# Alibaba-Gemini-Lab/Gemini-SEAL

Hardware: AMD Instinct MI355X
Metric: ciphertext multiply+relinearize/s (BFV N=2^15, 8 primes, bit-exact PARITY mode) (higher is better)
Workload: dtype u64

## Files before the change

gemini-seal_amd/csrc/devmath.hpp:

```cpp
#pragma once

#include <hip/hip_runtime.h>

#include <cstdint>
#include "ntt_bounds.hpp"

namespace sealhip
{
    using u64 = unsigned long long;

    struct PrimeDev
    {
        u64 p;
        u64 two_p;
        u64 rdp;
        u64 cr0, cr1;
        u64 inv_n, inv_n_shoup;
        u64 inv_n_w, inv_n_w_shoup;
        u64 ninv;
        const u64 *fwd;
        const u64 *inv;
        const double *fwd_d;
        const double *inv_d;
        double p_d, pinv_d;
    };

    constexpr double kTwo52 = 4503599627370496.0;
    __device__ __forceinline__ double fp_of(u64 bits)
    {
        return __longlong_as_double(static_cast<long long>(bits));
    }
    __device__ __forceinline__ u64 fp_bits(double v)
    {
        return static_cast<u64>(__double_as_longlong(v));
    }
    __device__ __forceinline__ double fp_from_u64(u64 x)
    {
        return fp_of(x | 0x4330000000000000ull) - kTwo52;
    }
    __device__ __forceinline__ u64 fp_to_u64(double r)
    {
        return fp_bits(r + kTwo52) & 0x000FFFFFFFFFFFFFull;
    }
    __device__ __forceinline__ double fp_reduce(double x, double p, double pinv)
    {
#pragma clang fp contract(off)
        return __builtin_fma(-__builtin_rint(x * pinv), p, x);
    }
    __device__ __forceinline__ double fp_canonical(double x, double p, double pinv)
    {
        const double r = fp_reduce(x, p, pinv);
        return r < 0.0 ? r + p : r;
    }
    __device__ __forceinline__ double fp_mulmod(double y, double w, double p, double pinv)
    {
#pragma clang fp contract(off)
        const double h = y * w;
        const double l = __builtin_fma(y, w, -h);
// ... 162 lines not shown
                : "v"(x0), "s"(s1), "v"(A)
                : "vcc");
        else
            asm("v_mad_u64_u32 %0, vcc, %2, %3, %4\n\ts_nop 1\n\tv_cndmask_b32_e64 %1, 0, 1, vcc"
                : "=&v"(B), "=&v"(cb)
                : "v"(x0), "v"(s1), "v"(A)
                : "vcc");
        const u64 addend = static_cast<u64>(static_cast<u32>(B >> 32)) | (static_cast<u64>(cb) << 32);
        return mad64<SU>(x1, s1, addend);
    }
    __device__ __forceinline__ u64 add_hi32(u64 v, u64 e)
    {
        u32 vh;
        asm("v_add_u32 %0, %1, %2" : "=v"(vh) : "v"(static_cast<u32>(v >> 32)), "v"(static_cast<u32>(e)));
        return static_cast<u64>(static_cast<u32>(v)) | (static_cast<u64>(vh) << 32);
    }
    template <bool WU>
    __device__ __forceinline__ u64 mullo2_acc(u64 acc, u64 x, u64 w, u64 q, u64 np)
    {
        const u32 x0 = static_cast<u32>(x), x1 = static_cast<u32>(x >> 32);
        const u32 w0 = static_cast<u32>(w), w1 = static_cast<u32>(w >> 32);
        const u32 q0 = static_cast<u32>(q), q1 = static_cast<u32>(q >> 32);
        const u32 n0 = static_cast<u32>(np), n1 = static_cast<u32>(np >> 32);
        u64 E = mul64<WU>(x0, w1);
        E = mad64<WU>(x1, w0, E);
        E = mad64<true>(q0, n1, E);
        E = mad64<true>(q1, n0, E);
        u64 V = mad64<WU>(x0, w0, acc);
        V = mad64<true>(q0, n0, V);
        return add_hi32(V, E);
    }
    __device__ __forceinline__ u64 mullo1_acc(u64 acc, u64 q, u64 np)
    {
        const u32 q0 = static_cast<u32>(q), q1 = static_cast<u32>(q >> 32);
        const u32 n0 = static_cast<u32>(np), n1 = static_cast<u32>(np >> 32);
        u64 E = mul64<true>(q0, n1);
        E = mad64<true>(q1, n0, E);
        return add_hi32(mad64<true>(q0, n0, acc), E);
    }
    template <bool WU>
    __device__ __forceinline__ u64 mulmod_lazy_hs(u64 x, u64 y, u64 yshoup, u64 neg_p)
    {
        return mullo2_acc<WU>(0, x, y, mulhi_c<WU>(x, yshoup), neg_p);
    }
    __device__ __forceinline__ u64 mulmod_shoup_hs(u64 x, u64 y, u64 yshoup, u64 p)
    {
        const u64 t = mulmod_lazy_hs<true>(x, y, yshoup, 0 - p);
        return t >= p ? t - p : t;
    }
    __device__ __forceinline__ u64 barrett_lazy_hs(u64 x, u64 rdp, u64 neg_p)
    {
        return mullo1_acc(x, mulhi_c<true>(x, rdp), neg_p);
    }
    __device__ __forceinline__ float small_quot_const(u64 p)
    {
        return static_cast<float>(4294967296.0 / static_cast<double>(p) * (1.0 - 0x1p-20));
    }
    __device__ __forceinline__ u64 reduce_small_quot(u64 x, float c, u64 neg_p)
    {
        float hf;
        asm("v_cvt_f32_u32 %0, %1" : "=v"(hf) : "v"(static_cast<u32>(x >> 32)));
        const u32 q = static_cast<u32>(hf * c);
        const u64 v = mad64<true>(q, static_cast<u32>(neg_p), x);
        return add_hi32(v, static_cast<u64>(q * static_cast<u32>(neg_p >> 32)));
    }
    template <bool SU>
    __device__ __forceinline__ u64 mulhi_apx(u64 x, u64 s)
    {
        const u32 x0 = static_cast<u32>(x), x1 = static_cast<u32>(x >> 32);
        const u32 s0 = static_cast<u32>(s), s1 = static_cast<u32>(s >> 32);
        const u64 A = mul64<SU>(x1, s0);
        u64 B;
        u32 cb;
        if (SU)
            asm("v_mad_u64_u32 %0, vcc, %2, %3, %4\n\ts_nop 1\n\tv_cndmask_b32_e64 %1, 0, 1, vcc"
                : "=&v"(B), "=&v"(cb)
                : "v"(x0), "s"(s1), "v"(A)
                : "vcc");
        else
            asm("v_mad_u64_u32 %0, vcc, %2, %3, %4\n\ts_nop 1\n\tv_cndmask_b32_e64 %1, 0, 1, vcc"
                : "=&v"(B), "=&v"(cb)
                : "v"(x0), "v"(s1), "v"(A)
                : "vcc");
        const u64 addend = static_cast<u64>(static_cast<u32>(B >> 32)) | (static_cast<u64>(cb) << 32);
        return mad64<SU>(x1, s1, addend);
    }
    template <int N>
    struct ZeroHi
    {
        u64 z[N];
        __device__ __forceinline__ void init()
        {
#pragma unroll
            for (int j = 0; j < N; j++)
            {
                u32 h;
                asm volatile("v_mov_b32 %0, 0" : "=v"(h));
                z[j] = static_cast<u64>(h) << 32;
            }
        }
    };
    __device__ __forceinline__ u64 with_low(u64 zp, u32 lo)
    {
        return (zp & 0xFFFFFFFF00000000ull) | lo;
    }
    template <bool SU>
// ... 351 lines not shown
```

gemini-seal_amd/csrc/engine.cpp:

```cpp
#include "engine.hpp"

#include <algorithm>
#include <atomic>
#include <cstdlib>
#include <cstring>

namespace sealhip
{
    namespace
    {
        template <class T>
        T *upload(Engine &e, std::vector<void *> &owned, const T *host, std::size_t count)
        {
            T *dev = nullptr;
            SEALHIP_CHECK(hipMalloc(reinterpret_cast<void **>(&dev), sizeof(T) * (count ? count : 1)));
            owned.push_back(dev);
            if (count)
                SEALHIP_CHECK(hipMemcpy(dev, host, sizeof(T) * count, hipMemcpyHostToDevice));
            (void)e;
            return dev;
        }

        RowMap make_map(const std::vector<unsigned short> &ids)
        {
// ... 477 lines not shown
                const u64 b = hr.Bsk[j];
                const HostNttTables &tb = tables[n_key + (j < B ? 2 + j : 0)];
                if (tb.p != b)
                    throw std::logic_error("internal: Bsk prime order");
                rd.floor_G1m_top[0][j] = mont(mulmod(rd.floor_G1[j], tb.inv_n, b), b);
                rd.floor_G1m_top[1][j] = mont(mulmod(rd.floor_G1[j], tb.inv_n_w, b), b);
                rd.floor_G1m_top[2][j] = mont(rd.floor_G1m_top[0][j], b);
                rd.floor_G1m_top[3][j] = mont(rd.floor_G1m_top[1][j], b);
                rd.b_p[j] = b;
                rd.b_w1[j] = tb.fwd.size() >= 4 ? tb.fwd[2] : 0;
                rd.b_w1s[j] = tb.fwd.size() >= 4 ? tb.fwd[3] : 0;
                rd.b_rdp[j] = tb.rdp ? tb.rdp : shoup(1, b);
                {
                    u64 inv = b;
                    for (int it = 0; it < 6; it++)
                        inv *= 2 - b * inv;
                    rd.b_ninv[j] = 0 - inv;
                }
            }
            for (int i = 0; i < k; i++)
            {
                const u64 qi = hr.q[i];
                rd.floor_F0_top[0][i] = mulmod(rd.floor_F0[i], tables[i].inv_n, qi);
                rd.floor_F0_top[1][i] = mulmod(rd.floor_F0[i], tables[i].inv_n_w, qi);
                rd.floor_F0_top_s[0][i] = shoup(rd.floor_F0_top[0][i], qi);
                rd.floor_F0_top_s[1][i] = shoup(rd.floor_F0_top[1][i], qi);
                for (int hh = 0; hh < 2; hh++)
                {
                    rd.floor_F0_top[2 + hh][i] = mont(rd.floor_F0_top[hh][i], qi);
                    rd.floor_F0_top_s[2 + hh][i] = shoup(rd.floor_F0_top[2 + hh][i], qi);
                }
                rd.q_p[i] = qi;
                rd.q_rdp[i] = tables[i].rdp ? tables[i].rdp : shoup(1, qi);
                {
                    u64 inv = qi;
                    for (int it = 0; it < 6; it++)
                        inv *= 2 - qi * inv;
                    rd.q_ninv[i] = 0 - inv;
                }
                rd.q_mt_inv_s[i] = shoup(rd.q_mt_inv[i], qi);
                rd.floor_F0_s[i] = shoup(rd.floor_F0[i], qi);
                rd.pBm[i] = mont(hr.prod_B_mod_q[i], qi);
                rd.nBm[i] = mont(qi - hr.prod_B_mod_q[i], qi);
                for (int j = 0; j < B; j++)
                    BQm[static_cast<std::size_t>(i) * B + j] = mont(hr.B_to_q.matrix[static_cast<std::size_t>(i) * B + j], qi);
            }
            for (int j = 0; j < B; j++)
                rd.B_to_mskm[j] = mont(hr.B_to_m_sk.matrix[j], hr.m_sk);
            rd.inv_prod_B_mod_msk_s = shoup(hr.inv_prod_B_mod_m_sk, hr.m_sk);
            rd.lift_L1m = upload<u64>(*this, lt.owned, L1m.data(), L1m.size());
            rd.floor_G2m = upload<u64>(*this, lt.owned, G2m.data(), G2m.size());
            rd.B_to_qm = upload<u64>(*this, lt.owned, BQm.data(), BQm.size());
            {
                HostBaseConv tg;
                tg.build(hr.q, std::vector<u64>{ t, hr.gamma });
                for (int i = 0; i < k; i++)
                {
                    const u64 qi = hr.q[i];
                    rd.dsr_scale[i] = mulmod(mulmod(t % qi, hr.gamma % qi, qi), tg.inv_punct[i], qi);
                    rd.dsr_scale_s[i] = shoup(rd.dsr_scale[i], qi);
                    rd.dsr_to_t[i] = tg.matrix[i];
                    rd.dsr_to_g[i] = tg.matrix[static_cast<std::size_t>(k) + i];
                }
                u64 pq_t = 1 % t, pq_g = 1;
                for (int i = 0; i < k; i++)
                {
                    pq_t = mulmod(pq_t, hr.q[i] % t, t);
                    pq_g = mulmod(pq_g, hr.q[i] % hr.gamma, hr.gamma);
                }
                u64 it = 0, ig = 0, igt = 0;
                if (!invmod(pq_t, t, it) || !invmod(pq_g, hr.gamma, ig) || !invmod(hr.gamma % t, t, igt))
                    throw std::logic_error("invalid rns bases");
                rd.dsr_neg_inv_q_t = it ? t - it : 0;
                rd.dsr_neg_inv_q_g = ig ? hr.gamma - ig : 0;
                rd.dsr_inv_gamma_t = igt;
                rd.dsr_gamma = hr.gamma;
                rd.gamma_prime = static_cast<unsigned>(n_key + 1);
            }
            rd.redc_small = bounds::behz_redc_small(k, B, max_q, max_b) ? 1 : 0;
        }
        lt.h_rns = rd;
        lt.d_rns = upload<RnsDev>(*this, lt.owned, &rd, 1);

        if (k <= k_first)
        {
            KsDev kd{};
            kd.k = k;
            kd.nsp = nsp;
            kd.nd = (k + nsp - 1) / nsp;
            kd.n_all = k_first;
            kd.n_total = n_key;
            kd.is_ckks = scheme == 2;
            kd.strict = mode_strict;
            const int rows = k + nsp;
            for (int r = 0; r < rows; r++)
                kd.row_prime[r] = static_cast<unsigned>(r < k ? r : k_first + (r - k));
            auto prime_of = [&](int r) { return key_moduli[kd.row_prime[r]]; };
            const std::size_t blk = static_cast<std::size_t>(2 * nsp + rows * nsp);
            std::vector<u64> modup(blk * kd.nd, 0);
            for (int j = 0; j < kd.nd; j++)
            {
                const int r0 = j * nsp, r1 = std::min(r0 + nsp, k), bs = r1 - r0;
                u64 *b = modup.data() + blk * j;
                for (int a = 0; a < bs; a++)
                {
                    const u64 pa = prime_of(r0 + a);
// ... 335 lines not shown
```

gemini-seal_amd/csrc/engine.hpp:

```cpp
#pragma once

#include <hip/hip_runtime.h>

#include <cstddef>
#include <array>
#include <atomic>
#include <cstdint>
#include <functional>
#include <map>
#include <memory>
#include <mutex>
#include <stdexcept>
#include <string>
#include <cstdlib>
#include <vector>

#include "devmath.hpp"
#include "ntt_bounds.hpp"
#include "hostmath.hpp"

namespace sealhip
{
    constexpr int kMaxRows = 136;
    constexpr int kMaxModuli = 64;
// ... 39 lines not shown
    constexpr int kNttTopDone = 0x80;
    constexpr int kNttDeferTop = 4;
    constexpr u64 kFpPrimeBound = u64(1) << bounds::kFpPrimeBits;

    struct NttRound
    {
        int beta, wlo, whi;
    };
    struct NttPass
    {
        int logn, t, c, b_lo, flags, nrounds;
        NttRound rounds[4];
    };
    struct NttPlan
    {
        int logn, npass, flags;
        bool serial;
        NttPass pass[2];
    };
    NttPlan plan_ntt(int logn, bool inverse, int flags);

    struct RnsDev
    {
        int k, nB, B;
        u64 t;
        u64 q_mt_inv[kMaxModuli];
        u64 q_inv[kMaxModuli];
        const u64 *q_to_Bsk;
        u64 q_to_mt[kMaxModuli];
        u64 inv_prod_q_mod_mt;
        u64 prod_q_mod_Bsk[kMaxModuli + 2], inv_prod_q_mod_Bsk[kMaxModuli + 2], inv_mt_mod_Bsk[kMaxModuli + 2];
        u64 B_inv[kMaxModuli + 1];
        const u64 *B_to_q;
        u64 B_to_msk[kMaxModuli + 1];
        u64 inv_prod_B_mod_msk;
        u64 prod_B_mod_q[kMaxModuli];
        u64 inv_q_last_mod_q[kMaxModuli];
        const u64 *lift_L1;
        const u64 *floor_G2;
        u64 lift_L2[kMaxModuli + 2];
        u64 floor_G1[kMaxModuli + 2];
        u64 floor_F0[kMaxModuli];
        u64 floor_F0_top[4][kMaxModuli], floor_F0_top_s[4][kMaxModuli];
        u64 floor_G1m_top[4][kMaxModuli + 2];
        u64 q_p[kMaxModuli], q_ninv[kMaxModuli], q_rdp[kMaxModuli];
        u64 b_p[kMaxModuli + 2], b_ninv[kMaxModuli + 2], b_rdp[kMaxModuli + 2];
        u64 b_w1[kMaxModuli + 2], b_w1s[kMaxModuli + 2];
        const u64 *lift_L1m, *floor_G2m, *B_to_qm;
        u64 lift_L2m[kMaxModuli + 2], floor_G1m[kMaxModuli + 2];
        u64 q_mt_inv_s[kMaxModuli], floor_F0_s[kMaxModuli];
        u64 B_to_mskm[kMaxModuli + 1];
        u64 inv_prod_B_mod_msk_s;
        u64 pBm[kMaxModuli], nBm[kMaxModuli];
        u64 dsr_scale[kMaxModuli], dsr_scale_s[kMaxModuli], dsr_to_t[kMaxModuli], dsr_to_g[kMaxModuli];
        u64 dsr_neg_inv_q_t, dsr_neg_inv_q_g, dsr_inv_gamma_t, dsr_gamma;
        unsigned gamma_prime;
        int redc_small;
        unsigned q_prime[kMaxModuli];
        unsigned bsk_prime[kMaxModuli + 2];
    };

    struct KsDev
    {
        int k, nsp, nd, n_all, n_total;
        int is_ckks, strict;
        unsigned row_prime[kMaxModuli];
        const u64 *modup;
        u64 inv_hat[kMaxModuli], inv_hat_shoup[kMaxModuli];
        const u64 *neg_hat;
        u64 invP[kMaxModuli], invP_shoup[kMaxModuli];
    };

    constexpr int kCkksMaxLimbs = 32;
    struct CkksDecodeDev
    {
        int k;
        u64 q[kCkksMaxLimbs];
        u64 half[kCkksMaxLimbs];
        u64 inv_punct[kCkksMaxLimbs];
        u64 punct[kCkksMaxLimbs * kCkksMaxLimbs];
    };

    struct NoiseBudgetDev
    {
        int k;
        u64 q[kMaxModuli];
        u64 half[kMaxModuli];
        u64 t_inv_punct[kMaxModuli];
        u64 punct[kMaxModuli * kMaxModuli];
    };

    struct LevelTools
    {
        std::unique_ptr<HostRnsTool> host_rns;
        RnsDev *d_rns = nullptr;
        KsDev *d_ks = nullptr;
        KsDev h_ks{};
        RnsDev h_rns{};
        std::vector<void *> owned;
        RowMap map_q{}, map_bsk{}, map_key{}, map_qbsk{};
    };

    struct KSwitchKey
    {
        u64 *d_data = nullptr;
        std::uint32_t n_digits = 0;
// ... 505 lines not shown
```

gemini-seal_amd/csrc/ntt_bounds.hpp:

```cpp
#pragma once
#include <cstdint>

namespace sealhip
{
    namespace bounds
    {
        using u64 = unsigned long long;
        using u128 = unsigned __int128;

        constexpr int kMinHalfLogn = 14, kMaxHalfLogn = 16;
        constexpr int kMaxPrimeBits = 61;
        constexpr u128 kWord = static_cast<u128>(1) << 64;
        constexpr long double kFpLimit = 9007199254740992.0L;

        constexpr u64 max_prime_of_bits(int bits)
        {
            return (bits >= 64 ? ~u64(0) : (u64(1) << bits) - 1);
        }
        constexpr u64 max_ntt_prime_of_bits(int bits, int logn)
        {
            return bits > logn + 1 ? (u64(1) << bits) - (u64(1) << (logn + 1)) + 1 : 0;
        }

        constexpr int kInvLazyProductMult = 4;
// ... 222 lines not shown
            }
            return peak;
        }
        constexpr int fp_prime_bits()
        {
            int bits = 0;
            for (int b = kMaxHalfLogn + 2; b <= 52; b++)
            {
                bool ok = true;
                for (int logn = kMinHalfLogn; logn <= kMaxHalfLogn; logn++)
                {
                    const long double p = static_cast<long double>(max_ntt_prime_of_bits(b, logn));
                    ok = ok && fp_fwd_peak(logn, p, 0x1p52L) < kFpLimit;
                    ok = ok && fp_inv_peak(logn - 1, p) < kFpLimit;
                    if (logn <= 15)
                        ok = ok && fp_inv_peak(logn, p) < kFpLimit;
                }
                if (ok)
                    bits = b;
            }
            return bits;
        }
        constexpr int kFpPrimeBits = fp_prime_bits();
        static_assert(kFpPrimeBits == 50, "FP64 instances: primes below 2^50 (and raw inputs below 2^52)");
        constexpr u64 kFpInputBound = u64(1) << 52;
        constexpr bool fp_admits(u64 p)
        {
            return p <= max_prime_of_bits(kFpPrimeBits);
        }
        constexpr bool dotacc_ok(int nterms, int bits)
        {
            if (nterms < 1 || bits < 33 || bits > 64)
                return false;
            const u128 lim = kWord;
            const int nm = (2 * nterms + 7) / 8;
            const int per_m = (2 * nterms + nm - 1) / nm;
            const u128 low = static_cast<u128>(nterms) << 48;
            const u128 mid = static_cast<u128>(per_m) << bits;
            const u128 high = static_cast<u128>(nterms) << (2 * (bits - 32));
            return low <= lim && mid <= lim && high <= lim;
        }
        constexpr int kDotAccOperandBits = 61;
        constexpr int dotacc_max_terms()
        {
            int n = 0;
            for (int t = 1; t <= 4096; t++)
                if (dotacc_ok(t, kDotAccOperandBits))
                    n = t;
                else
                    break;
            return n;
        }
        static_assert(dotacc_max_terms() >= 64, "DotAcc on 61-bit operands: at least 64 terms (the kernels use up to k + 2 <= 34)");

        constexpr bool small_quot_admits(u64 p, int mult)
        {
            if (p < kSmallQuotMinPrime || mult < 1 || mult > 128 || static_cast<u128>(mult) * p > kWord)
                return false;
            const long double loss = 0x1p32L / static_cast<long double>(p) +
                                     static_cast<long double>(mult) * (0x1p-20L + 3 * 0x1p-24L + 0x1p-51L);
            return loss <= 0.5L;
        }

        constexpr bool behz_redc_small(int k, int B, u64 max_q, u64 max_b)
        {
            const u128 s1 = static_cast<u128>(k) * max_q + 2 * static_cast<u128>(max_b);
            const u128 s2 = static_cast<u128>(B + 1) * max_b;
            return k >= 1 && B >= 1 && s1 <= kWord && s2 <= kWord;
        }
        static_assert(!behz_redc_small(15, 16, u64(1) << 40, (u64(1) << 60) - (u64(1) << 55)),
                      "s2 at |B| = 16 for every m_sk");
        constexpr int kBehzExactMaxK = 15;
    }
}
```

gemini-seal_amd/csrc/rns.hip:

```cpp
#include <type_traits>

#include "engine.hpp"

namespace sealhip
{
    namespace
    {
        template <int N, int I = 0, class F>
        __device__ __forceinline__ void static_for(F &&f)
        {
            if constexpr (I < N)
            {
                f(std::integral_constant<int, I>{});
                static_for<N, I + 1>(f);
            }
        }

        template <class T>
        __device__ __forceinline__ const __attribute__((address_space(4))) T *kc(const T *p)
        {
            return (const __attribute__((address_space(4))) T *)p;
        }

        struct Cols
        {
            std::size_t item, c;
        };
        __device__ __forceinline__ bool column(std::size_t count, int logn, Cols &out)
        {
            const std::size_t i = blockIdx.x * static_cast<std::size_t>(blockDim.x) + threadIdx.x;
            out.item = i >> logn;
            out.c = i & ((static_cast<std::size_t>(1) << logn) - 1);
            return out.item < count;
        }

        template <int KMAX>
        __device__ __forceinline__ u64 dot_mod(const u64 (&t)[KMAX], int k, const u64 *__restrict__ mrow,
                                               const PrimeDev &P)
        {
            u64 lo = 0, hi = 0;
#pragma unroll
            for (int i = 0; i < KMAX; i++)
                if (i < k)
                    mac128(lo, hi, t[i], mrow[i]);
            return barrett_reduce_128(lo, hi, P.p, P.cr0, P.cr1);
        }

        template <int KMAX>
        __global__ __launch_bounds__(kThreads) void fastbconv_m_tilde_kernel(
            const RnsDev *__restrict__ d, const PrimeDev *__restrict__ primes, const u64 *__restrict__ in,
            std::size_t in_stride, u64 *__restrict__ out, std::size_t out_stride, std::size_t count, int logn)
        {
            Cols cc;
            if (!column(count, logn, cc))
                return;
            const int k = d->k, nB = d->nB;
            const std::size_t N = static_cast<std::size_t>(1) << logn;
            const u64 *pin = in + cc.item * in_stride + cc.c;
            u64 *pout = out + cc.item * out_stride + cc.c;
            u64 t[KMAX];
#pragma unroll
            for (int i = 0; i < KMAX; i++)
                if (i < k)
                {
                    const PrimeDev &Q = primes[d->q_prime[i]];
                    t[i] = mul_mod(pin[i * N], d->q_mt_inv[i], Q.p, Q.cr0, Q.cr1);
                }
            for (int j = 0; j < nB; j++)
                pout[j * N] = dot_mod<KMAX>(t, k, d->q_to_Bsk + j * k, primes[d->bsk_prime[j]]);
            u64 acc = 0;
#pragma unroll
            for (int i = 0; i < KMAX; i++)
                if (i < k)
                    acc += t[i] * d->q_to_mt[i];
// ... 55 lines not shown
                {
                    const PrimeDev &Q = primes[d->q_prime[i]];
                    t[i] = mul_mod(pin[i * N], d->q_mt_inv[i], Q.p, Q.cr0, Q.cr1);
                    acc += t[i] * d->q_to_mt[i];
                }
            const u64 r_mt = r_m_tilde(acc & 0xFFFFFFFFull, d);
            for (int j = 0; j < nB; j++)
            {
                const PrimeDev &Bp = primes[d->bsk_prime[j]];
                const u64 conv = dot_mod<KMAX>(t, k, d->q_to_Bsk + j * k, Bp);
                pout[j * N] = sm_mrq_one(conv, r_mt, d, j, Bp);
            }
        }

        template <int KMAX, bool TOP = false>
        __global__ __launch_bounds__(kThreads) void bfv_lift2_kernel(const RnsDev *__restrict__ d_,
                                                                     const PrimeDev *__restrict__ primes_,
                                                                     const u64 *__restrict__ in, std::size_t in_stride,
                                                                     u64 *__restrict__ out, std::size_t out_stride,
                                                                     std::size_t count, int logn)
        {
            static_assert(!TOP || KMAX < 0, "the paired-column form exists for the exact-K instances");
            Cols cc;
            if (!column(count, TOP ? logn - 1 : logn, cc))
                return;
            constexpr int KA = KMAX < 0 ? -KMAX : KMAX;
            constexpr int NC = TOP ? 2 : 1;
            const auto *d = kc(d_);
            const auto *primes = kc(primes_);
            const int k = KMAX < 0 ? KA : d->k, nB = d->nB;
            const std::size_t N = static_cast<std::size_t>(1) << logn;
            const u64 *pin = in + cc.item * in_stride + cc.c;
            u64 *pout = out + cc.item * out_stride + cc.c;
            u64 t[NC][KA];
            u64 acc[NC] = {};
            (void)primes;
#pragma unroll
            for (int i = 0; i < KA; i++)
                if (KMAX < 0 || i < k)
                {
                    const u64 qp = d->q_p[i];
#pragma unroll
                    for (int h = 0; h < NC; h++)
                    {
                        t[h][i] = mulmod_shoup_hs(pin[i * N + h * (N >> 1)], d->q_mt_inv[i], d->q_mt_inv_s[i], qp);
                        acc[h] += t[h][i] * d->q_to_mt[i];
                    }
                }
            u64 r_mt[NC];
#pragma unroll
            for (int h = 0; h < NC; h++)
                r_mt[h] = r_m_tilde(acc[h] & 0xFFFFFFFFull, d);
            const bool small = KMAX < 0 ? true : d->redc_small != 0;
            SplitT ts[NC][KA];
            if constexpr (KMAX < 0)
                static_for<KA>([&](auto I) {
#pragma unroll
                    for (int h = 0; h < NC; h++)
                        ts[h][I.value] = SplitT(t[h][I.value]);
                });
            const auto *L1m = kc(d->lift_L1m);
            const auto *L2m = kc(d->lift_L2m);
            const auto row_out = [&](int j) {
                const u64 bp = d->b_p[j];
                const auto *row = L1m + j * k;
                u64 v[NC];
#pragma unroll
                for (int h = 0; h < NC; h++)
                {
                    u64 temp = r_mt[h];
                    if (temp >= (1ull << 31))
                        temp += bp - (1ull << 32);
                    u64 lo, hi;
                    if constexpr (KMAX < 0)
                    {
                        DotAcc<KA + 1> acc2;
                        acc2.template add<0>(SplitT(temp), L2m[j]);
                        static_for<KA>([&](auto I) { acc2.template add<I.value + 1>(ts[h][I.value], row[I.value]); });
                        acc2.finish(lo, hi);
                    }
                    else
                    {
                        lo = temp * L2m[j];
                        hi = mulhi(temp, L2m[j]);
#pragma unroll
                        for (int i = 0; i < KA; i++)
                            if (i < k)
                                mac128(lo, hi, t[h][i], row[i]);
                    }
                    v[h] = redc_finish(redc128(lo, hi, bp, d->b_ninv[j]), bp, d->b_rdp[j], small);
                }
                if constexpr (TOP)
                {
                    butterfly_fwd_hs<true>(v[0], v[1], d->b_w1[j], d->b_w1s[j], 0 - bp, bp << 1);
                    pout[j * N + (N >> 1)] = v[1];
                }
                pout[j * N] = v[0];
            };
            if constexpr (KMAX < 0)
            {
                static_for<KA + 1>([&](auto J) { row_out(J.value); });
                if (nB == KA + 2)
                    row_out(KA + 1);
            }
            else
                for (int j = 0; j < nB; j++)
                    row_out(j);
        }

        template <class PP>
        __device__ __forceinline__ u64 after_top(u64 u, u64 v, bool is_hi, PP P)
        {
            const u64 p = P->p, two_p = P->two_p, neg_p = 0 - p;
            u64 r;
            if (is_hi)
                r = mulmod_lazy_hs<true>(u - v + two_p, P->inv_n_w, P->inv_n_w_shoup, neg_p);
            else
            {
                u64 tt = u + v;
                tt = tt >= two_p ? tt - two_p : tt;
                r = mulmod_lazy_hs<true>(tt, P->inv_n, P->inv_n_shoup, neg_p);
            }
            return r >= p ? r - p : r;
        }
        template <bool REDUCE>
        __device__ __forceinline__ u64 before_top(u64 u, u64 v, bool is_hi, u64 two_p)
        {
            const u64 vv = is_hi ? two_p - v : v;
            u64 r = u + vv;
            if (REDUCE)
                r = r >= two_p ? r - two_p : r;
            return r;
        }
        template <int KMAX, bool DEFER>
        __global__ __launch_bounds__(kThreads) void bfv_floor_sk2_kernel(const RnsDev *__restrict__ d_,
                                                                         const PrimeDev *__restrict__ primes_,
                                                                         const u64 *__restrict__ in,
                                                                         std::size_t in_stride, u64 *__restrict__ out,
                                                                         std::size_t out_stride, std::size_t count,
                                                                         int logn, int mont, unsigned *__restrict__ tflags)
        {
            constexpr int KA = KMAX < 0 ? -KMAX : KMAX;
            const std::size_t N = static_cast<std::size_t>(1) << logn;
// ... 1 lines not shown
            Cols cc;
            bool is_hi = false;
            if constexpr (DEFER)
            {
                const std::size_t per_item = N / kThreads, bid = blockIdx.x;
                cc.item = bid / per_item;
                if (cc.item >= count)
                    return;
                const unsigned pl = static_cast<unsigned>(bid - cc.item * per_item), r = pl & 15u;
                is_hi = (r >> 3) != 0;
                cc.c = (is_hi ? half : 0) + static_cast<std::size_t>(((pl >> 4) << 3) | (r & 7u)) * kThreads + threadIdx.x;
            }
            else if (!column(count, logn, cc))
                return;
            const auto *d = kc(d_);
            const auto *primes = kc(primes_);
            const int k = KMAX < 0 ? KA : d->k, B = d->B;
            const bool extraB = B > KA;
            auto lt_B = [&](int j) { return KMAX < 0 ? (j < KA || (j == KA && extraB)) : j < B; };
            auto le_B = [&](int j) { return KMAX < 0 ? (j <= KA || (j == KA + 1 && extraB)) : j <= B; };
            const u64 *pin = in + cc.item * in_stride + cc.c;
            const u64 *pitem = in + cc.item * in_stride;
            const std::size_t c_lo = cc.c & (half - 1);
            u64 *pout = out + cc.item * out_stride + cc.c;
            u64 ru[2 * KA + 2], rv[2 * KA + 2];
#pragma unroll
            for (int i = 0; i < KA; i++)
                if (KMAX < 0 || i < k)
                {
                    ru[i] = DEFER ? pitem[i * N + c_lo] : pin[i * N];
                    rv[i] = DEFER ? pitem[i * N + c_lo + half] : 0;
                }
            const auto load_bsk = [&](int j) {
                if (le_B(j))
                {
                    ru[KA + j] = DEFER ? pitem[(k + j) * N + c_lo] : pin[(k + j) * N];
                    rv[KA + j] = DEFER ? pitem[(k + j) * N + c_lo + half] : 0;
                }
            };
            if constexpr (KMAX < 0)
                static_for<KA + 2>([&](auto J) { load_bsk(J.value); });
            else
            {
#pragma unroll
                for (int j = 0; j < KA + 2; j++)
                    load_bsk(j);
            }
            __builtin_amdgcn_sched_barrier(0);
            u64 t[KA];
            const int top_sel = (mont ? 2 : 0) + (is_hi ? 1 : 0);
            const auto *F0t = DEFER ? kc(d->floor_F0_top[top_sel]) : kc(d->floor_F0);
            const auto *F0ts = DEFER ? kc(d->floor_F0_top_s[top_sel]) : kc(d->floor_F0_s);
            (void)primes;
            u64 cF0[KA], cF0s[KA], cQ[KA];
#pragma unroll
            for (int i = 0; i < KA; i++)
                if (KMAX < 0 || i < k)
                {
                    cF0[i] = F0t[i];
                    cF0s[i] = F0ts[i];
                    cQ[i] = d->q_p[i];
                }
            __builtin_amdgcn_sched_barrier(0);
#pragma unroll
            for (int i = 0; i < KA; i++)
                if (KMAX < 0 || i < k)
                {
                    const u64 qp = cQ[i];
                    if (DEFER)
                        t[i] = mulmod_shoup_hs(before_top<false>(ru[i], rv[i], is_hi, qp << 1), cF0[i], cF0s[i], qp);
                    else
                        t[i] = mulmod_shoup_hs(ru[i], cF0[i], cF0s[i], qp);
                }
            u64 tb[KA + 1];
            u64 fl_sk = 0;
            const bool small = KMAX < 0 ? true : d->redc_small != 0;
            SplitT ts[KA], tbs[KA + 1];
            if constexpr (KMAX < 0)
                static_for<KA>([&](auto I) { ts[I.value] = SplitT(t[I.value]); });
            const auto *G1m = DEFER ? kc(d->floor_G1m_top[top_sel]) : kc(d->floor_G1m);
            const auto *G2m = kc(d->floor_G2m);
            const auto bsk_row = [&](int j) {
                if (le_B(j))
                {
                    const u64 bp = d->b_p[j];
                    const auto *row = G2m + j * k;
                    const u64 x = DEFER ? before_top<true>(ru[KA + j], rv[KA + j], is_hi, bp << 1) : ru[KA + j];
                    u64 lo, hi;
                    if constexpr (KMAX < 0)
                    {
                        DotAcc<KA + 1> acc2;
                        acc2.template add<0>(SplitT(x), G1m[j]);
                        static_for<KA>([&](auto I) { acc2.template add<I.value + 1>(ts[I.value], row[I.value]); });
                        acc2.finish(lo, hi);
                    }
                    else
                    {
                        lo = x * G1m[j];
                        hi = mulhi(x, G1m[j]);
#pragma unroll
                        for (int i = 0; i < KA; i++)
                            if (i < k)
                                mac128(lo, hi, t[i], row[i]);
                    }
                    const u64 v = redc_finish(redc128(lo, hi, bp, d->b_ninv[j]), bp, d->b_rdp[j], small);
                    if (lt_B(j))
                        tb[j < KA + 1 ? j : 0] = v;
                    else
                        fl_sk = v;
                    __builtin_amdgcn_sched_barrier(0);
                }
            };
            if constexpr (KMAX < 0)
                static_for<KA + 2>([&](auto J) { bsk_row(J.value); });
            else
                for (int j = 0; j < KA + 2; j++)
                    bsk_row(j);
            const u64 mp = d->b_p[B];
            const auto *BtoMsk = kc(d->B_to_mskm);
            u64 lo = 0, hi = 0;
            if constexpr (KMAX < 0)
            {
                static_for<KA + 1>([&](auto J) {
                    if (lt_B(J.value))
                        tbs[J.value] = SplitT(tb[J.value]);
                });
                DotAcc<KA + 1> acc2;
                static_for<KA + 1>([&](auto J) {
                    if (lt_B(J.value))
                        acc2.template add<J.value>(tbs[J.value], BtoMsk[J.value]);
                });
                acc2.finish(lo, hi);
            }
            else
            {
#pragma unroll
                for (int j = 0; j < KA + 1; j++)
                    if (lt_B(j))
                        mac128(lo, hi, tb[j], BtoMsk[j]);
            }
            const u64 conv_sk = redc_finish(redc128(lo, hi, mp, d->b_ninv[B]), mp, d->b_rdp[B], small);
            const u64 alpha = mulmod_shoup(conv_sk + (mp - fl_sk), d->inv_prod_B_mod_msk, d->inv_prod_B_mod_msk_s, mp);
            const bool neg = alpha > (mp >> 1);
            const u64 a2 = neg ? mp - alpha : alpha;
            const SplitT a2s(a2);
            const auto *pBm = kc(d->pBm);
            const auto *nBm = kc(d->nBm);
            const auto *BtoQ = kc(d->B_to_qm);
            u64 nz = 0;
            const auto q_row = [&](int i) {
                const u64 c = neg ? pBm[i] : nBm[i];
                const auto *mrow = BtoQ + i * B;
                u64 l2, h2;
                if constexpr (KMAX < 0)
                {
                    DotAcc<KA + 2> acc2;
                    acc2.template add<0>(a2s, c);
                    static_for<KA + 1>([&](auto J) {
                        if (lt_B(J.value))
                            acc2.template add<J.value + 1>(tbs[J.value], mrow[J.value]);
                    });
                    acc2.finish(l2, h2);
                }
                else
                {
                    l2 = a2 * c;
                    h2 = mulhi(a2, c);
#pragma unroll
                    for (int j = 0; j < KA + 1; j++)
                        if (lt_B(j))
                            mac128(l2, h2, tb[j], mrow[j]);
                }
                const u64 qp = d->q_p[i];
                const u64 w = redc_finish(redc128(l2, h2, qp, d->q_ninv[i]), qp, d->q_rdp[i], small);
                pout[i * N] = w;
                nz |= w;
                __builtin_amdgcn_sched_barrier(0);
            };
            if constexpr (KMAX < 0)
                static_for<KA>([&](auto I) { q_row(I.value); });
            else
                for (int i = 0; i < k; i++)
                    q_row(i);
            note_nonzero(tflags, cc.item, nz);
        }

        template <int KMAX>
        __global__ __launch_bounds__(kThreads) void fast_floor_kernel(const RnsDev *__restrict__ d,
                                                                      const PrimeDev *__restrict__ primes,
                                                                      const u64 *__restrict__ in, std::size_t in_stride,
                                                                      u64 *__restrict__ out, std::size_t out_stride,
                                                                      std::size_t count, int logn, int mul_t)
        {
            Cols cc;
            if (!column(count, logn, cc))
                return;
            const int k = d->k, nB = d->nB;
            const std::size_t N = static_cast<std::size_t>(1) << logn;
            const u64 *pin = in + cc.item * in_stride + cc.c;
            u64 *pout = out + cc.item * out_stride + cc.c;
            u64 t[KMAX];
#pragma unroll
            for (int i = 0; i < KMAX; i++)
                if (i < k)
                {
                    const PrimeDev &Q = primes[d->q_prime[i]];
                    u64 x = pin[i * N];
                    if (mul_t)
                        x = mul_mod(x, d->t, Q.p, Q.cr0, Q.cr1);
                    t[i] = mul_mod(x, d->q_inv[i], Q.p, Q.cr0, Q.cr1);
                }
            for (int j = 0; j < nB; j++)
            {
                const PrimeDev &Bp = primes[d->bsk_prime[j]];
                const u64 conv = dot_mod<KMAX>(t, k, d->q_to_Bsk + j * k, Bp);
                u64 x = pin[(k + j) * N];
                if (mul_t)
                    x = mul_mod(x, d->t, Bp.p, Bp.cr0, Bp.cr1);
                pout[j * N] = mul_mod(x + (Bp.p - conv), d->inv_prod_q_mod_Bsk[j], Bp.p, Bp.cr0, Bp.cr1);
            }
        }

        template <int KMAX>
        __device__ __forceinline__ void sk_finish(const RnsDev *d, const PrimeDev *primes, const u64 (&tb)[KMAX + 1],
                                                  u64 in_sk, u64 *pout, std::size_t N)
        {
            const int k = d->k, B = d->B;
// ... 460 lines not shown
```

Before: 23270.

## Use 31-bit split dot accumulators and packed constant rows in BEHZ conversions

Replaces the 32-bit split DotAcc with a 31-bit split accumulator (DotAcc31) whose constants are prepacked, so partial products stay carry-free in fewer registers. It also adds an exact Montgomery reduction with a single conditional correction, and lays out per-row constants (lift/floor matrices, prime, ninv) contiguously in device tables that are read through scalar-register windows. The goal is fewer carry-handling instructions and fewer scattered scalar loads in the lift and floor base-conversion kernels, at the cost of extra device tables and new overflow bounds that must hold.

```diff
diff --git a/gemini-seal_amd/csrc/devmath.hpp b/gemini-seal_amd/csrc/devmath.hpp
--- a/gemini-seal_amd/csrc/devmath.hpp
+++ b/gemini-seal_amd/csrc/devmath.hpp
@@ -4,6 +4,7 @@
 
 #include <cstdint>
 #include "ntt_bounds.hpp"
+#include "dotacc.hpp"
 
 namespace sealhip
 {
@@ -272,6 +273,12 @@
     {
         return mullo1_acc(x, mulhi_c<true>(x, rdp), neg_p);
     }
+    __device__ __forceinline__ u64 redc_canonical_hs(u64 lo, u64 hi, u64 p, u64 ninv)
+    {
+        const u64 m = mullo1_acc(0, lo, 0 - ninv);
+        const u64 dd = hi - mulhi_c<true>(m, p);
+        return static_cast<long long>(dd) < 0 ? dd + p : dd;
+    }
     __device__ __forceinline__ float small_quot_const(u64 p)
     {
         return static_cast<float>(4294967296.0 / static_cast<double>(p) * (1.0 - 0x1p-20));
diff --git a/gemini-seal_amd/csrc/dotacc.hpp b/gemini-seal_amd/csrc/dotacc.hpp
--- /dev/null
+++ b/gemini-seal_amd/csrc/dotacc.hpp
@@ -0,0 +1,65 @@
+#pragma once
+
+#include "ntt_bounds.hpp"
+
+#if defined(__HIPCC__)
+#define SEALHIP_HD __host__ __device__ __forceinline__
+#else
+#define SEALHIP_HD inline
+#endif
+
+namespace sealhip
+{
+    constexpr unsigned long long dot31_pack(unsigned long long c)
+    {
+        return ((c >> 31) << 32) | (c & 0x7FFFFFFFull);
+    }
+    constexpr unsigned long long dot31_unpack(unsigned long long pk)
+    {
+        return ((pk >> 32) << 31) | (pk & 0xFFFFFFFFull);
+    }
+
+    struct Split31
+    {
+        unsigned t0, t1;
+        SEALHIP_HD Split31() : t0(0), t1(0) {}
+        SEALHIP_HD explicit Split31(unsigned long long t)
+            : t0(static_cast<unsigned>(t) & 0x7FFFFFFFu), t1(static_cast<unsigned>(t >> 31))
+        {}
+    };
+
+    template <int NTERMS>
+    struct DotAcc31
+    {
+        static_assert(bounds::dotacc31_ok(NTERMS, bounds::kDotAccOperandBits),
+                      "carry-free accumulators: NTERMS products of 61-bit operands must fit (ntt_bounds.hpp section 5)");
+        using u64 = unsigned long long;
+        static constexpr int NL = bounds::dotacc31_nl(NTERMS), NM = bounds::dotacc31_nm(NTERMS),
+                             NH = bounds::dotacc31_nh(NTERMS);
+        u64 l[NL] = {}, m[NM] = {}, h[NH] = {};
+        template <int IDX>
+        SEALHIP_HD void add(const Split31 &t, u64 cpk)
+        {
+            static_assert(IDX >= 0 && IDX < NTERMS, "term index");
+            const unsigned c0 = static_cast<unsigned>(cpk), c1 = static_cast<unsigned>(cpk >> 32);
+            l[IDX % NL] += static_cast<u64>(t.t0) * c0;
+            m[(2 * IDX) % NM] += static_cast<u64>(t.t0) * c1;
+            m[(2 * IDX + 1) % NM] += static_cast<u64>(t.t1) * c0;
+            h[IDX % NH] += static_cast<u64>(t.t1) * c1;
+        }
+        SEALHIP_HD void finish(u64 &lo, u64 &hi) const
+        {
+            typedef unsigned __int128 u128;
+            u128 s = m[0], r = l[0];
+            for (int i = 1; i < NM; i++)
+                s += m[i];
+            for (int i = 0; i < NH; i++)
+                s += static_cast<u128>(h[i]) << 31;
+            for (int i = 1; i < NL; i++)
+                r += l[i];
+            r += s << 31;
+            lo = static_cast<u64>(r);
+            hi = static_cast<u64>(r >> 64);
+        }
+    };
+}
diff --git a/gemini-seal_amd/csrc/engine.cpp b/gemini-seal_amd/csrc/engine.cpp
--- a/gemini-seal_amd/csrc/engine.cpp
+++ b/gemini-seal_amd/csrc/engine.cpp
@@ -553,6 +553,51 @@
             rd.floor_G2m = upload<u64>(*this, lt.owned, G2m.data(), G2m.size());
             rd.B_to_qm = upload<u64>(*this, lt.owned, BQm.data(), BQm.size());
             {
+                const std::size_t ls = static_cast<std::size_t>(k) + 3, qs = static_cast<std::size_t>(B) + 4;
+                std::vector<u64> lrows(nB * ls), frows(5 * nB * ls), qrows(k * qs), first(5 * static_cast<std::size_t>(k) * 3);
+                for (int j = 0; j < nB; j++)
+                {
+                    u64 *lr = &lrows[j * ls];
+                    lr[0] = dot31_pack(rd.lift_L2m[j]);
+                    for (int i = 0; i < k; i++)
+                        lr[1 + i] = dot31_pack(L1m[static_cast<std::size_t>(j) * k + i]);
+                    lr[k + 1] = rd.b_p[j];
+                    lr[k + 2] = rd.b_ninv[j];
+                    for (int sel = 0; sel < 5; sel++)
+                    {
+                        u64 *fr = &frows[(static_cast<std::size_t>(sel) * nB + j) * ls];
+                        fr[0] = dot31_pack(sel < 4 ? rd.floor_G1m_top[sel][j] : rd.floor_G1m[j]);
+                        for (int i = 0; i < k; i++)
+                            fr[1 + i] = dot31_pack(G2m[static_cast<std::size_t>(j) * k + i]);
+                        fr[k + 1] = rd.b_p[j];
+                        fr[k + 2] = rd.b_ninv[j];
+                    }
+                }
+                for (int i = 0; i < k; i++)
+                {
+                    u64 *qr = &qrows[i * qs];
+                    qr[0] = dot31_pack(rd.pBm[i]);
+                    qr[1] = dot31_pack(rd.nBm[i]);
+                    for (int j = 0; j < B; j++)
+                        qr[2 + j] = dot31_pack(BQm[static_cast<std::size_t>(i) * B + j]);
+                    qr[B + 2] = rd.q_p[i];
+                    qr[B + 3] = rd.q_ninv[i];
+                    for (int sel = 0; sel < 5; sel++)
+                    {
+                        u64 *f = &first[(static_cast<std::size_t>(sel) * k + i) * 3];
+                        f[0] = sel < 4 ? rd.floor_F0_top[sel][i] : rd.floor_F0[i];
+                        f[1] = sel < 4 ? rd.floor_F0_top_s[sel][i] : rd.floor_F0_s[i];
+                        f[2] = rd.q_p[i];
+                    }
+                }
+                for (int j = 0; j < B; j++)
+                    rd.B_to_mskp[j] = dot31_pack(rd.B_to_mskm[j]);
+                rd.lift_rows = upload<u64>(*this, lt.owned, lrows.data(), lrows.size());
+                rd.floor_rows = upload<u64>(*this, lt.owned, frows.data(), frows.size());
+                rd.q_rows = upload<u64>(*this, lt.owned, qrows.data(), qrows.size());
+                rd.floor_first = upload<u64>(*this, lt.owned, first.data(), first.size());
+            }
+            {
                 HostBaseConv tg;
                 tg.build(hr.q, std::vector<u64>{ t, hr.gamma });
                 for (int i = 0; i < k; i++)
diff --git a/gemini-seal_amd/csrc/engine.hpp b/gemini-seal_amd/csrc/engine.hpp
--- a/gemini-seal_amd/csrc/engine.hpp
+++ b/gemini-seal_amd/csrc/engine.hpp
@@ -115,6 +115,11 @@
         u64 B_to_mskm[kMaxModuli + 1];
         u64 inv_prod_B_mod_msk_s;
         u64 pBm[kMaxModuli], nBm[kMaxModuli];
+        const u64 *lift_rows;
+        const u64 *floor_rows;
+        const u64 *q_rows;
+        const u64 *floor_first;
+        u64 B_to_mskp[kMaxModuli + 1];
         u64 dsr_scale[kMaxModuli], dsr_scale_s[kMaxModuli], dsr_to_t[kMaxModuli], dsr_to_g[kMaxModuli];
         u64 dsr_neg_inv_q_t, dsr_neg_inv_q_g, dsr_inv_gamma_t, dsr_gamma;
         unsigned gamma_prime;
diff --git a/gemini-seal_amd/csrc/ntt_bounds.hpp b/gemini-seal_amd/csrc/ntt_bounds.hpp
--- a/gemini-seal_amd/csrc/ntt_bounds.hpp
+++ b/gemini-seal_amd/csrc/ntt_bounds.hpp
@@ -298,6 +298,28 @@
             return n;
         }
         static_assert(dotacc_max_terms() >= 64, "DotAcc on 61-bit operands: at least 64 terms (the kernels use up to k + 2 <= 34)");
+        constexpr int dotacc31_nl(int nterms) { return (nterms + 3) / 4; }
+        constexpr int dotacc31_nm(int nterms) { return (2 * nterms + 7) / 8; }
+        constexpr int dotacc31_nh(int nterms) { return (nterms + 15) / 16; }
+        constexpr bool dotacc31_ok(int nterms, int bits)
+        {
+            if (nterms < 1 || nterms > 64 || bits < 32 || bits > 62)
+                return false;
+            const u128 lim = kWord;
+            const int nl = dotacc31_nl(nterms), nm = dotacc31_nm(nterms), nh = dotacc31_nh(nterms);
+            const u128 low = static_cast<u128>((nterms + nl - 1) / nl) << 62;
+            const u128 mid = static_cast<u128>((2 * nterms + nm - 1) / nm) << bits;
+            const u128 high = static_cast<u128>((nterms + nh - 1) / nh) << (2 * (bits - 31));
+            const bool sum_fits = 2 * bits + 6 <= 128;
+            return low <= lim && mid <= lim && high <= lim && sum_fits;
+        }
+        constexpr bool dotacc31_all_ok(int max_terms)
+        {
+            for (int t = 1; t <= max_terms; t++)
+                if (!dotacc31_ok(t, kDotAccOperandBits))
+                    return false;
+            return true;
+        }
 
         constexpr bool small_quot_admits(u64 p, int mult)
         {
@@ -317,5 +339,7 @@
         static_assert(!behz_redc_small(15, 16, u64(1) << 40, (u64(1) << 60) - (u64(1) << 55)),
                       "s2 at |B| = 16 for every m_sk");
         constexpr int kBehzExactMaxK = 15;
+        static_assert(dotacc31_all_ok(kBehzExactMaxK + 2),
+                      "DotAcc31 on 61-bit operands: every term count of the exact-k instances (up to k + 2)");
     }
 }
diff --git a/gemini-seal_amd/csrc/rns.hip b/gemini-seal_amd/csrc/rns.hip
--- a/gemini-seal_amd/csrc/rns.hip
+++ b/gemini-seal_amd/csrc/rns.hip
@@ -20,6 +20,18 @@
         __device__ __forceinline__ const __attribute__((address_space(4))) T *kc(const T *p)
         {
             return (const __attribute__((address_space(4))) T *)p;
+        }
+
+        template <class T>
+        __device__ __forceinline__ const __attribute__((address_space(4))) T *row_window(
+            const __attribute__((address_space(4))) T *row)
+        {
+            asm volatile("" : "+s"(row));
+            return row;
+        }
+        __device__ __forceinline__ void row_done(u64 &v)
+        {
+            asm volatile("" : "+v"(v));
         }
 
         struct Cols
@@ -181,18 +193,22 @@
             for (int h = 0; h < NC; h++)
                 r_mt[h] = r_m_tilde(acc[h] & 0xFFFFFFFFull, d);
             const bool small = KMAX < 0 ? true : d->redc_small != 0;
-            SplitT ts[NC][KA];
+            Split31 ts[NC][KA];
             if constexpr (KMAX < 0)
                 static_for<KA>([&](auto I) {
 #pragma unroll
                     for (int h = 0; h < NC; h++)
-                        ts[h][I.value] = SplitT(t[h][I.value]);
+                        ts[h][I.value] = Split31(t[h][I.value]);
                 });
             const auto *L1m = kc(d->lift_L1m);
             const auto *L2m = kc(d->lift_L2m);
+            const auto *Lrows = kc(d->lift_rows);
             const auto row_out = [&](int j) {
-                const u64 bp = d->b_p[j];
-                const auto *row = L1m + j * k;
+                auto *row = KMAX < 0 ? Lrows + j * (KA + 3) : L1m + j * k;
+                if constexpr (KMAX < 0)
+                    row = row_window(row);
+                const u64 bp = KMAX < 0 ? row[KA + 1] : d->b_p[j];
+                const u64 ninv = KMAX < 0 ? row[KA + 2] : d->b_ninv[j];
                 u64 v[NC];
 #pragma unroll
                 for (int h = 0; h < NC; h++)
@@ -203,9 +219,9 @@
                     u64 lo, hi;
                     if constexpr (KMAX < 0)
                     {
-                        DotAcc<KA + 1> acc2;
-                        acc2.template add<0>(SplitT(temp), L2m[j]);
-                        static_for<KA>([&](auto I) { acc2.template add<I.value + 1>(ts[h][I.value], row[I.value]); });
+                        DotAcc31<KA + 1> acc2;
+                        acc2.template add<0>(Split31(temp), row[0]);
+                        static_for<KA>([&](auto I) { acc2.template add<I.value + 1>(ts[h][I.value], row[I.value + 1]); });
                         acc2.finish(lo, hi);
                     }
                     else
@@ -217,7 +233,10 @@
                             if (i < k)
                                 mac128(lo, hi, t[h][i], row[i]);
                     }
-                    v[h] = redc_finish(redc128(lo, hi, bp, d->b_ninv[j]), bp, d->b_rdp[j], small);
+                    if constexpr (KMAX < 0)
+                        v[h] = redc_canonical_hs(lo, hi, bp, ninv);
+                    else
+                        v[h] = redc_finish(redc128(lo, hi, bp, ninv), bp, d->b_rdp[j], small);
                 }
                 if constexpr (TOP)
                 {
@@ -325,46 +344,42 @@
             const auto *F0t = DEFER ? kc(d->floor_F0_top[top_sel]) : kc(d->floor_F0);
             const auto *F0ts = DEFER ? kc(d->floor_F0_top_s[top_sel]) : kc(d->floor_F0_s);
             (void)primes;
-            u64 cF0[KA], cF0s[KA], cQ[KA];
+            const auto *first = kc(d->floor_first) + (DEFER ? top_sel : 4) * (KA * 3);
 #pragma unroll
             for (int i = 0; i < KA; i++)
                 if (KMAX < 0 || i < k)
                 {
-                    cF0[i] = F0t[i];
-                    cF0s[i] = F0ts[i];
-                    cQ[i] = d->q_p[i];
-                }
-            __builtin_amdgcn_sched_barrier(0);
-#pragma unroll
-            for (int i = 0; i < KA; i++)
-                if (KMAX < 0 || i < k)
-                {
-                    const u64 qp = cQ[i];
+                    const u64 cF0 = KMAX < 0 ? first[3 * i] : F0t[i], cF0s = KMAX < 0 ? first[3 * i + 1] : F0ts[i];
+                    const u64 qp = KMAX < 0 ? first[3 * i + 2] : d->q_p[i];
                     if (DEFER)
-                        t[i] = mulmod_shoup_hs(before_top<false>(ru[i], rv[i], is_hi, qp << 1), cF0[i], cF0s[i], qp);
+                        t[i] = mulmod_shoup_hs(before_top<false>(ru[i], rv[i], is_hi, qp << 1), cF0, cF0s, qp);
                     else
-                        t[i] = mulmod_shoup_hs(ru[i], cF0[i], cF0s[i], qp);
+                        t[i] = mulmod_shoup_hs(ru[i], cF0, cF0s, qp);
                 }
             u64 tb[KA + 1];
             u64 fl_sk = 0;
             const bool small = KMAX < 0 ? true : d->redc_small != 0;
-            SplitT ts[KA], tbs[KA + 1];
+            Split31 ts[KA], tbs[KA + 1];
             if constexpr (KMAX < 0)
-                static_for<KA>([&](auto I) { ts[I.value] = SplitT(t[I.value]); });
+                static_for<KA>([&](auto I) { ts[I.value] = Split31(t[I.value]); });
             const auto *G1m = DEFER ? kc(d->floor_G1m_top[top_sel]) : kc(d->floor_G1m);
             const auto *G2m = kc(d->floor_G2m);
+            const auto *Frows = kc(d->floor_rows) + (DEFER ? top_sel : 4) * (d->nB * (KA + 3));
             const auto bsk_row = [&](int j) {
                 if (le_B(j))
                 {
-                    const u64 bp = d->b_p[j];
-                    const auto *row = G2m + j * k;
+                    auto *row = KMAX < 0 ? Frows + j * (KA + 3) : G2m + j * k;
+                    if constexpr (KMAX < 0)
+                        row = row_window(row);
+                    const u64 bp = KMAX < 0 ? row[KA + 1] : d->b_p[j];
+                    const u64 ninv = KMAX < 0 ? row[KA + 2] : d->b_ninv[j];
                     const u64 x = DEFER ? before_top<true>(ru[KA + j], rv[KA + j], is_hi, bp << 1) : ru[KA + j];
                     u64 lo, hi;
                     if constexpr (KMAX < 0)
                     {
-                        DotAcc<KA + 1> acc2;
-                        acc2.template add<0>(SplitT(x), G1m[j]);
-                        static_for<KA>([&](auto I) { acc2.template add<I.value + 1>(ts[I.value], row[I.value]); });
+                        DotAcc31<KA + 1> acc2;
+                        acc2.template add<0>(Split31(x), row[0]);
+                        static_for<KA>([&](auto I) { acc2.template add<I.value + 1>(ts[I.value], row[I.value + 1]); });
                         acc2.finish(lo, hi);
                     }
                     else
@@ -376,7 +391,13 @@
                             if (i < k)
                                 mac128(lo, hi, t[i], row[i]);
                     }
-                    const u64 v = redc_finish(redc128(lo, hi, bp, d->b_ninv[j]), bp, d->b_rdp[j], small);
+                    u64 v;
+                    if constexpr (KMAX < 0)
+                        v = redc_canonical_hs(lo, hi, bp, ninv);
+                    else
+                        v = redc_finish(redc128(lo, hi, bp, ninv), bp, d->b_rdp[j], small);
+                    if constexpr (KMAX < 0)
+                        row_done(v);
                     if (lt_B(j))
                         tb[j < KA + 1 ? j : 0] = v;
                     else
@@ -390,15 +411,15 @@
                 for (int j = 0; j < KA + 2; j++)
                     bsk_row(j);
             const u64 mp = d->b_p[B];
-            const auto *BtoMsk = kc(d->B_to_mskm);
+            const auto *BtoMsk = KMAX < 0 ? kc(d->B_to_mskp) : kc(d->B_to_mskm);
             u64 lo = 0, hi = 0;
             if constexpr (KMAX < 0)
             {
                 static_for<KA + 1>([&](auto J) {
                     if (lt_B(J.value))
-                        tbs[J.value] = SplitT(tb[J.value]);
+                        tbs[J.value] = Split31(tb[J.value]);
                 });
-                DotAcc<KA + 1> acc2;
+                DotAcc31<KA + 1> acc2;
                 static_for<KA + 1>([&](auto J) {
                     if (lt_B(J.value))
                         acc2.template add<J.value>(tbs[J.value], BtoMsk[J.value]);
@@ -412,22 +433,25 @@
                     if (lt_B(j))
                         mac128(lo, hi, tb[j], BtoMsk[j]);
             }
-            const u64 conv_sk = redc_finish(redc128(lo, hi, mp, d->b_ninv[B]), mp, d->b_rdp[B], small);
+            const u64 conv_sk = KMAX < 0 ? redc_canonical_hs(lo, hi, mp, d->b_ninv[B])
+                                         : redc_finish(redc128(lo, hi, mp, d->b_ninv[B]), mp, d->b_rdp[B], small);
             const u64 alpha = mulmod_shoup(conv_sk + (mp - fl_sk), d->inv_prod_B_mod_msk, d->inv_prod_B_mod_msk_s, mp);
             const bool neg = alpha > (mp >> 1);
             const u64 a2 = neg ? mp - alpha : alpha;
-            const SplitT a2s(a2);
+            const Split31 a2s(a2);
             const auto *pBm = kc(d->pBm);
             const auto *nBm = kc(d->nBm);
             const auto *BtoQ = kc(d->B_to_qm);
+            const auto *Qrows = kc(d->q_rows);
             u64 nz = 0;
             const auto q_row = [&](int i) {
-                const u64 c = neg ? pBm[i] : nBm[i];
-                const auto *mrow = BtoQ + i * B;
+                const auto *qrow = Qrows + i * (B + 4);
+                const u64 c = KMAX < 0 ? (neg ? qrow[0] : qrow[1]) : (neg ? pBm[i] : nBm[i]);
+                const auto *mrow = KMAX < 0 ? qrow + 2 : BtoQ + i * B;
                 u64 l2, h2;
                 if constexpr (KMAX < 0)
                 {
-                    DotAcc<KA + 2> acc2;
+                    DotAcc31<KA + 2> acc2;
                     acc2.template add<0>(a2s, c);
                     static_for<KA + 1>([&](auto J) {
                         if (lt_B(J.value))
@@ -444,8 +468,12 @@
                         if (lt_B(j))
                             mac128(l2, h2, tb[j], mrow[j]);
                 }
-                const u64 qp = d->q_p[i];
-                const u64 w = redc_finish(redc128(l2, h2, qp, d->q_ninv[i]), qp, d->q_rdp[i], small);
+                const u64 qp = KMAX < 0 ? qrow[B + 2] : d->q_p[i];
+                u64 w;
+                if constexpr (KMAX < 0)
+                    w = redc_canonical_hs(l2, h2, qp, qrow[B + 3]);
+                else
+                    w = redc_finish(redc128(l2, h2, qp, d->q_ninv[i]), qp, d->q_rdp[i], small);
                 pout[i * N] = w;
                 nz |= w;
                 __builtin_amdgcn_sched_barrier(0);
```

Result: faster. 23750, median of 6 (+2.0%).
